# kmurf1999/RustSolver

Measured on NVIDIA B200. Metric: cfr_iterations_per_sec, higher is better.
Workload: dtype f32

## Files before the change

rustsolver_b200/csrc/kernels.cu:

```cuda
#include "kernels.cuh"

#ifndef RS_MIN_BLOCKS_288
#define RS_MIN_BLOCKS_288 3
#endif
#ifndef RS_MIN_BLOCKS_352
#define RS_MIN_BLOCKS_352 2
#endif

#ifndef RS_POLL_SLEEP_NS
#define RS_POLL_SLEEP_NS 64
#endif

namespace rs {

namespace {

__device__ __forceinline__ uint32_t ld_acquire_u32(const uint32_t* p) {
    uint32_t v;
    asm volatile("ld.acquire.gpu.global.u32 %0, [%1];" : "=r"(v) : "l"(p) : "memory");
    return v;
}
__device__ __forceinline__ uint32_t ld_acquire_sys_u32(const uint32_t* p) {
    uint32_t v;
    asm volatile("ld.acquire.sys.global.u32 %0, [%1];" : "=r"(v) : "l"(p) : "memory");
// ... 42 lines not shown
        : "=r"(ok)
        : "r"(uint32_t(__cvta_generic_to_shared(bar))), "r"(parity)
        : "memory");
    return ok != 0;
}

__device__ __forceinline__ bool wait_gives_up(const TaskArgs& A, unsigned long long t_start, uint32_t& spins) {
    if ((++spins & 255u) != 0) return false;
    if (*reinterpret_cast<const volatile unsigned int*>(&A.ctl->abort)) return true;
    bool trip = false;
    if ((spins & 4095u) == 0 && A.host_abort && *A.host_abort) trip = true;
    if (A.wait_timeout_ns) {
        unsigned long long now;
        asm volatile("mov.u64 %0, %globaltimer;" : "=l"(now));
        if (now - t_start > A.wait_timeout_ns) trip = true;
    }
    if (trip) atomicExch(&A.ctl->abort, 1u);
    return trip;
}
__device__ __forceinline__ unsigned long long global_ns() {
    unsigned long long now;
    asm volatile("mov.u64 %0, %globaltimer;" : "=l"(now));
    return now;
}

struct Ctx {
    int nc;
    int tid, lane, warp, nwarps;
    int pos4;
    int p, o, Hp, Ho, HpP, HoP, Hx;
};

constexpr int HCAP = MAX_TASK_THREADS * 4;
extern __shared__ __align__(16) float smem_raw[];
#define SM_RS (smem_raw)
#define SM_P (smem_raw + HCAP)
#define SM_GB (smem_raw + 2 * HCAP + 4)
#define SM_WSA (smem_raw + 4 * HCAP + 12)
#define SM_WSB (smem_raw + 4 * HCAP + 44)
#define SM_B (smem_raw + 4 * HCAP + 76)
#define SM_REC (reinterpret_cast<uint32_t*>(smem_raw + 4 * HCAP + 140))
#define SM_CL (reinterpret_cast<uint32_t*>(smem_raw + 8 * HCAP + 140))
#define SM_X (smem_raw + 9 * HCAP + 140)

__device__ __forceinline__ void stage_lists_raw(int tid, int HoP, const uint16_t* __restrict__ cl_pos_b) {
    if (8 * tid < 2 * HoP)
        asm volatile("cp.async.cg.shared.global [%0], [%1], 16;" ::"r"(uint32_t(__cvta_generic_to_shared(SM_CL + 4 * tid))), "l"(cl_pos_b + 8 * tid)
                     : "memory");
    asm volatile("cp.async.commit_group;" ::: "memory");
}

__device__ __forceinline__ float scan_reach(const Ctx& c, const float* r) {
    csync(c.nc);
    float4 x = f4zero();
    if (c.pos4 < c.HoP) x = *reinterpret_cast<const float4*>(r + c.pos4);
    float y[8];
    uint32_t w[4];
    {
        asm volatile("cp.async.wait_group 0;" ::: "memory");
        uint4 u = make_uint4(0x07ff07ffu, 0x07ff07ffu, 0x07ff07ffu, 0x07ff07ffu);
        if (8 * c.tid < 2 * c.HoP) u = *reinterpret_cast<const uint4*>(SM_CL + 4 * c.tid);
        w[0] = u.x;
        w[1] = u.y;
        w[2] = u.z;
        w[3] = u.w;
#pragma unroll
        for (int i = 0; i < 4; ++i) {
            const uint32_t a = w[i] & CL_POS_MASK, b = (w[i] >> 16) & CL_POS_MASK;
            y[2 * i] = a != CL_POS_NONE ? r[a] : 0.f;
            y[2 * i + 1] = b != CL_POS_NONE ? r[b] : 0.f;
        }
    }
    const float la = (x.x + x.y) + (x.z + x.w);
    float lb = 0.f;
#pragma unroll
    for (int i = 0; i < 8; ++i) lb += y[i];
    float ia = la, ib = lb;
#pragma unroll
    for (int d = 1; d < 32; d <<= 1) {
        const float ta = __shfl_up_sync(0xffffffffu, ia, d);
        const float tb = __shfl_up_sync(0xffffffffu, ib, d);
        if (c.lane >= d) {
            ia += ta;
            ib += tb;
        }
    }
    if (c.lane == 31) {
        SM_WSA[c.warp] = ia;
        SM_WSB[c.warp] = ib;
    }
    csync(c.nc);
    float wa = c.lane < c.nwarps ? SM_WSA[c.lane] : 0.f;
    float wb = c.lane < c.nwarps ? SM_WSB[c.lane] : 0.f;
#pragma unroll
    for (int d = 1; d < 16; d <<= 1) {
        const float ta = __shfl_up_sync(0xffffffffu, wa, d);
        const float tb = __shfl_up_sync(0xffffffffu, wb, d);
        if (c.lane >= d) {
            wa += ta;
            wb += tb;
        }
    }
    const float total = __shfl_sync(0xffffffffu, wa, c.nwarps - 1);
    const float total_b = __shfl_sync(0xffffffffu, wb, c.nwarps - 1);
    const float base_a = c.warp > 0 ? __shfl_sync(0xffffffffu, wa, c.warp - 1) : 0.f;
    const float base_b = c.warp > 0 ? __shfl_sync(0xffffffffu, wb, c.warp - 1) : 0.f;
    float ea = base_a + ia - la, eb = base_b + ib - lb;
    if (c.pos4 < c.HoP) {
        float4 o;
        o.x = ea;
        o.y = ea + x.x;
        o.z = o.y + x.y;
        o.w = o.z + x.z;
        *reinterpret_cast<float4*>(SM_P + c.pos4) = o;
    }
    if (8 * c.tid < 2 * c.HoP) {
        float4 o0, o1;
        o0.x = eb;
        o0.y = o0.x + y[0];
        o0.z = o0.y + y[1];
        o0.w = o0.z + y[2];
        o1.x = o0.w + y[3];
        o1.y = o1.x + y[4];
        o1.z = o1.y + y[5];
        o1.w = o1.z + y[6];
        *reinterpret_cast<float4*>(SM_GB + 8 * c.tid) = o0;
        *reinterpret_cast<float4*>(SM_GB + 8 * c.tid + 4) = o1;
        const uint32_t ord0 = ((w[0] >> 11) & 7u) | (((w[0] >> 27) & 7u) << 3);
        float* bp = SM_B + (c.tid == 0 ? 0u : ord0);
        const float ex[8] = {o0.x, o0.y, o0.z, o0.w, o1.x, o1.y, o1.z, o1.w};
#pragma unroll
        for (int i = 0; i < 8; ++i) {
            const bool first = ((w[i >> 1] >> ((i & 1) * 16)) & CL_FIRST) != 0;
            if (first) *bp++ = ex[i];
        }
        if (c.tid == 0) SM_B[ord0] = total_b;
    }
    if (c.tid == 0) {
        SM_P[c.HoP] = total;
        SM_GB[2 * c.HoP] = total_b;
    }
    csync(c.nc);
    return total;
}

__device__ __forceinline__ void load_recs4(const uint32_t* __restrict__ planes, int HpP, int pos4, uint4 (&rec)[4]) {
    const uint4 w0 = __ldg(reinterpret_cast<const uint4*>(planes + pos4));
    const uint4 w1 = __ldg(reinterpret_cast<const uint4*>(planes + HpP + pos4));
    const uint4 w2 = __ldg(reinterpret_cast<const uint4*>(planes + 2 * HpP + pos4));
    const uint4 w3 = __ldg(reinterpret_cast<const uint4*>(planes + 3 * HpP + pos4));
    rec[0] = make_uint4(w0.x, w1.x, w2.x, w3.x);
    rec[1] = make_uint4(w0.y, w1.y, w2.y, w3.y);
    rec[2] = make_uint4(w0.z, w1.z, w2.z, w3.z);
    rec[3] = make_uint4(w0.w, w1.w, w2.w, w3.w);
}

__device__ __forceinline__ void stage_recs(const Ctx& c, const uint32_t* __restrict__ planes) {
    if (c.pos4 < c.HpP) {
#pragma unroll
        for (int w = 0; w < 4; ++w)
            asm volatile("cp.async.cg.shared.global [%0], [%1], 16;" ::"r"(uint32_t(__cvta_generic_to_shared(SM_REC + w * HCAP + c.pos4))),
                         "l"(planes + size_t(w) * c.HpP + c.pos4)
                         : "memory");
    }
    asm volatile("cp.async.commit_group;" ::: "memory");
}
__device__ __forceinline__ void staged_recs_wait() { asm volatile("cp.async.wait_group 0;" ::: "memory"); }
__device__ __forceinline__ void staged_recs4(const Ctx& c, uint4 (&rec)[4]) {
    const uint4 w0 = *reinterpret_cast<const uint4*>(SM_REC + c.pos4);
    const uint4 w1 = *reinterpret_cast<const uint4*>(SM_REC + HCAP + c.pos4);
    const uint4 w2 = *reinterpret_cast<const uint4*>(SM_REC + 2 * HCAP + c.pos4);
    const uint4 w3 = *reinterpret_cast<const uint4*>(SM_REC + 3 * HCAP + c.pos4);
    rec[0] = make_uint4(w0.x, w1.x, w2.x, w3.x);
    rec[1] = make_uint4(w0.y, w1.y, w2.y, w3.y);
    rec[2] = make_uint4(w0.z, w1.z, w2.z, w3.z);
    rec[3] = make_uint4(w0.w, w1.w, w2.w, w3.w);
}

__device__ __forceinline__ float ldsb(const float* base, uint32_t byte_off) {
    return *reinterpret_cast<const float*>(reinterpret_cast<const char*>(base) + byte_off);
}
__device__ __forceinline__ void hand_terms(const Ctx& c, const float* r, float total, const uint4& rec, float& mass, float& sd) {
    const uint32_t k0 = rec.w & 0x1ffu, k1 = (rec.w >> 9) & 0x1ffu, same4 = rec.w >> 18;
    const float g0s = ldsb(SM_B, k0), g0e = ldsb(SM_B + 1, k0), g1s = ldsb(SM_B, k1), g1e = ldsb(SM_B + 1, k1);
    mass = total - (g0e - g0s) - (g1e - g1s) + (same4 != HREC_SAME_NONE ? ldsb(r, same4) : 0.f);
    sd = ldsb(SM_P, rec.x & 0xffffu) + ldsb(SM_P, rec.x >> 16) - total - ldsb(SM_GB, rec.y & 0xffffu) - ldsb(SM_GB, rec.y >> 16) + g0s + g0e -
         ldsb(SM_GB, rec.z & 0xffffu) - ldsb(SM_GB, rec.z >> 16) + g1s + g1e;
}
__device__ __forceinline__ float hand_mass(const Ctx& c, const float* r, float total, const uint4& rec) {
    const uint32_t k0 = rec.w & 0x1ffu, k1 = (rec.w >> 9) & 0x1ffu, same4 = rec.w >> 18;
    return total - (ldsb(SM_B + 1, k0) - ldsb(SM_B, k0)) - (ldsb(SM_B + 1, k1) - ldsb(SM_B, k1)) + (same4 != HREC_SAME_NONE ? ldsb(r, same4) : 0.f);
}

__device__ __forceinline__ float4 load_reach4(const TaskArgs& A, const Ctx& c, const NodeTask& nt, const RoundArgs& Rk, int k, int b) {
    float4 r = f4zero();
    if (c.pos4 >= c.HoP) return r;
    if (nt.r_in == RIN_INITIAL) {
        const uint32_t nl = Rk.rp[c.o].n_live[b];
        uint32_t s[4];
        unpack4(__ldg(reinterpret_cast<const uint2*>(Rk.rp[c.o].slot_of_pos + size_t(b) * c.HoP + c.pos4)), s);
        const float* __restrict__ w = A.root_weights[c.o];
#pragma unroll
        for (int i = 0; i < 4; ++i) f4set(r, i, uint32_t(c.pos4 + i) < nl ? __ldg(w + s[i]) : 0.f);
    } else if (nt.rin_parent_round) {
        const RoundArgs& Rp = A.rounds[k - 1];
        const float* src = Rp.rbuf + (size_t(nt.r_in) * Rp.n_boards + Rk.parent_board[b]) * c.HoP;
        uint32_t pp[4];
        unpack4(__ldg(reinterpret_cast<const uint2*>(Rk.rp[c.o].parent_pos + size_t(b) * c.HoP + c.pos4)), pp);
#pragma unroll
        for (int i = 0; i < 4; ++i) f4set(r, i, pp[i] != 0xffffu ? __ldcg(src + pp[i]) : 0.f);
    } else {
        r = ldcg4(Rk.rbuf + (size_t(nt.r_in) * Rk.n_boards + b) * c.HoP + c.pos4);
    }
    return r;
}

__device__ __forceinline__ float4 child_value4(const TaskArgs& A, const Ctx& c, const RoundArgs& Rk, const TaskChild& ch, int b) {
    float4 v = f4zero();
    if (c.pos4 >= c.HpP) return v;
    for (int s = 0; s < ch.n_src; ++s) {
        const TaskSrc sr = A.srcs[ch.src_first + s];
        const float* base = (sr.kind == SK_CBUF ? Rk.cbuf : Rk.gathered) + (size_t(sr.buf) * Rk.n_boards + b) * c.HpP;
        v = f4add(v, ldcg4(base + c.pos4));
    }
// ... 46 lines not shown
                g[4 * v + 1] = t.y;
                g[4 * v + 2] = t.z;
                g[4 * v + 3] = t.w;
            }
        } else {
#pragma unroll
            for (int e = 0; e < 4 * NA; ++e) g[e] = 0.f;
        }
    } else {
#pragma unroll
        for (int i = 0; i < 4; ++i)
#pragma unroll
            for (int a = 0; a < NA; ++a) g[i * NA + a] = rows[i] != 0xffffu ? slab[size_t(rows[i]) * NA + a] : 0.f;
    }
}

template <int NA>
__device__ __forceinline__ void xs_pick(const TaskArgs& A, float u, float (&sg)[NA]) {
    int pick = NA - 1;
    bool found = false;
    float cum = 0.f;
#pragma unroll
    for (int a = 0; a + 1 < NA; ++a) {
        cum += sg[a];
        if (!found && u < cum) {
            pick = a;
            found = true;
        }
    }
#pragma unroll
    for (int a = 0; a < NA; ++a) sg[a] = (a == pick) ? (A.xs_mode == 2 ? sg[a] : 1.0f) : 0.f;
}

template <int MODE, int NA, bool XS>
__device__ __forceinline__ void task_down(const TaskArgs& A, const Ctx& c, const NodeTask& nt, const RoundArgs& Rk, int k, int b) {
    const DevRoundPlayer& O = Rk.rp[c.o];
    const uint32_t nrp = O.n_rows_pad[b];
    const float* __restrict__ slab = (MODE == KM_CFR ? O.regrets : O.ssum) + O.board_off[b] + size_t(nrp) * nt.cum_a;
    if (nt.out >= 0) {
        stage_lists_raw(c.tid, c.HoP, O.cl_pos + size_t(b) * 2 * c.HoP);
        stage_recs(c, reinterpret_cast<const uint32_t*>(Rk.rp[c.p].hrec) + size_t(b) * 4 * c.HpP);
    }
    const float4 r4 = load_reach4(A, c, nt, Rk, k, b);
    uint32_t rows[4] = {0xffffu, 0xffffu, 0xffffu, 0xffffu};
    if (!O.identity && c.pos4 < c.HoP) unpack4(__ldg(reinterpret_cast<const uint2*>(O.row_of_pos + size_t(b) * c.HoP + c.pos4)), rows);
    float g[4 * NA];
    load_rows<NA>(slab, O.identity != 0, c.pos4, nrp, rows, g);
    float4 v[NA];
    uint32_t xs_slot[4] = {0, 0, 0, 0};
    if (XS && c.pos4 < c.HoP) unpack4(__ldg(reinterpret_cast<const uint2*>(O.slot_of_pos + size_t(b) * c.HoP + c.pos4)), xs_slot);
#pragma unroll
    for (int i = 0; i < 4; ++i) {
        float sg[NA];
        sigma_row<NA>(g, i, sg);
        if (XS) xs_pick<NA>(A, xs_uniform(A.xs_key, nt.an_index, uint32_t(Rk.board_base + b), xs_slot[i]), sg);
        const float r = f4get(r4, i);
#pragma unroll
        for (int a = 0; a < NA; ++a) f4set(v[a], i, r * sg[a]);
    }
    int slot = 0;
#pragma unroll
    for (int a = 0; a < NA; ++a) {
        const int ck = nt.child[a].kind;
        if (c.pos4 < c.HoP) {
            if (ck == CK_FOLD || ck == CK_SHOWDOWN) *reinterpret_cast<float4*>(SM_X + slot * c.Hx + c.pos4) = v[a];
            else if (nt.child[a].buf >= 0) stcg4(Rk.rbuf + (size_t(nt.child[a].buf) * Rk.n_boards + b) * c.HoP + c.pos4, v[a]);
        }
        if (ck == CK_FOLD || ck == CK_SHOWDOWN) ++slot;
    }
    if (nt.out < 0) return;
    const DevRoundPlayer& Pp = Rk.rp[c.p];
    const uint32_t nl_p = Pp.n_live[b];
    const float scale = Rk.chance_scale[b];
    float4 acc = f4zero();
    slot = 0;
    for (int a = 0; a < NA; ++a) {
        const int ck = nt.child[a].kind;
        if (ck != CK_FOLD && ck != CK_SHOWDOWN) continue;
        const float* r = SM_X + slot * c.Hx;
        ++slot;
        const float cf = nt.child[a].coef * scale;
        const float total = scan_reach(c, r);
        staged_recs_wait();
        if (c.pos4 < c.HpP) {
            uint4 rec[4];
            staged_recs4(c, rec);
#pragma unroll
            for (int i = 0; i < 4; ++i) {
                if (uint32_t(c.pos4 + i) < nl_p) {
                    float m, sd;
                    if (ck == CK_FOLD) {
                        m = hand_mass(c, r, total, rec[i]);
                        f4set(acc, i, f4get(acc, i) + cf * m);
                    } else {
                        hand_terms(c, r, total, rec[i], m, sd);
                        f4set(acc, i, f4get(acc, i) + cf * sd);
                    }
                }
            }
        }
    }
    if (c.pos4 < c.HpP) stcg4(Rk.cbuf + (size_t(nt.out) * Rk.n_boards + b) * c.HpP + c.pos4, acc);
}

template <int MODE, bool XS>
__device__ __forceinline__ void task_down_generic(const TaskArgs& A, const Ctx& c, const NodeTask& nt, const RoundArgs& Rk, int k, int b) {
    const DevRoundPlayer& O = Rk.rp[c.o];
    const uint32_t nrp = O.n_rows_pad[b];
    const float* __restrict__ slab = (MODE == KM_CFR ? O.regrets : O.ssum) + O.board_off[b] + size_t(nrp) * nt.cum_a;
    const float4 r4 = load_reach4(A, c, nt, Rk, k, b);
    const int n_act = nt.n_act;
    const uint32_t nl_o = O.n_live[b];
    uint32_t rows[4] = {0xffffu, 0xffffu, 0xffffu, 0xffffu};
    if (c.pos4 < c.HoP) unpack4(__ldg(reinterpret_cast<const uint2*>(O.row_of_pos + size_t(b) * c.HoP + c.pos4)), rows);
    if (c.pos4 < c.HoP) {
        for (int i = 0; i < 4; ++i) {
            const bool live = uint32_t(c.pos4 + i) < nl_o && rows[i] != 0xffffu;
            const float r = live ? f4get(r4, i) : 0.f;
            float norm = 0.f;
            if (live)
                for (int a = 0; a < n_act; ++a) norm += fmaxf(slab[size_t(rows[i]) * n_act + a], 0.f);
            int pick = -1;
            if (XS && live) {
                const float u = xs_uniform(A.xs_key, nt.an_index, uint32_t(Rk.board_base + b), O.slot_of_pos[size_t(b) * c.HoP + c.pos4 + i]);
                pick = n_act - 1;
                float cum = 0.f;
                for (int a = 0; a + 1 < n_act; ++a) {
                    cum += norm > 0.f ? fmaxf(slab[size_t(rows[i]) * n_act + a], 0.f) / norm : 1.0f / float(n_act);
                    if (u < cum) {
                        pick = a;
                        break;
                    }
                }
            }
            int slot = 0;
            for (int a = 0; a < n_act; ++a) {
                float v = 0.f;
                if (live) v = norm > 0.f ? r * fmaxf(slab[size_t(rows[i]) * n_act + a], 0.f) / norm : r / float(n_act);
                if (XS && live) v = (a == pick) ? (A.xs_mode == 2 ? v : r) : 0.f;
                const int ck = nt.child[a].kind;
                if (ck == CK_FOLD || ck == CK_SHOWDOWN) SM_X[(slot++) * c.Hx + c.pos4 + i] = v;
                else if (nt.child[a].buf >= 0) __stcg(Rk.rbuf + (size_t(nt.child[a].buf) * Rk.n_boards + b) * c.HoP + c.pos4 + i, v);
            }
        }
    }
    if (nt.out < 0) return;
    const DevRoundPlayer& Pp = Rk.rp[c.p];
    const uint32_t nl_p = Pp.n_live[b];
    const float scale = Rk.chance_scale[b];
    stage_lists_raw(c.tid, c.HoP, O.cl_pos + size_t(b) * 2 * c.HoP);
    float4 acc = f4zero();
    uint4 rec[4];
    if (c.pos4 < c.HpP) load_recs4(reinterpret_cast<const uint32_t*>(Pp.hrec) + size_t(b) * 4 * c.HpP, c.HpP, c.pos4, rec);
    int slot = 0;
    for (int a = 0; a < n_act; ++a) {
        const int ck = nt.child[a].kind;
        if (ck != CK_FOLD && ck != CK_SHOWDOWN) continue;
        const float* r = SM_X + slot * c.Hx;
        ++slot;
        const float cf = nt.child[a].coef * scale;
        const float total = scan_reach(c, r);
        if (c.pos4 < c.HpP) {
#pragma unroll
            for (int i = 0; i < 4; ++i) {
                if (uint32_t(c.pos4 + i) < nl_p) {
                    float m, sd;
                    hand_terms(c, r, total, rec[i], m, sd);
                    f4set(acc, i, f4get(acc, i) + cf * (ck == CK_FOLD ? m : sd));
                }
            }
        }
    }
    if (c.pos4 < c.HpP) stcg4(Rk.cbuf + (size_t(nt.out) * Rk.n_boards + b) * c.HpP + c.pos4, acc);
}

__device__ __forceinline__ void trav_terms(const TaskArgs& A, const Ctx& c, const NodeTask& nt, const RoundArgs& Rk, int k, int b,
                                           bool need_sd, float4& mass, float4& sd) {
    const DevRoundPlayer& Pp = Rk.rp[c.p];
    stage_lists_raw(c.tid, c.HoP, Rk.rp[c.o].cl_pos + size_t(b) * 2 * c.HoP);
    stage_recs(c, reinterpret_cast<const uint32_t*>(Pp.hrec) + size_t(b) * 4 * c.HpP);
    const float4 r4 = load_reach4(A, c, nt, Rk, k, b);
    if (c.pos4 < c.HoP) *reinterpret_cast<float4*>(SM_RS + c.pos4) = r4;
    const float total = scan_reach(c, SM_RS);
    mass = f4zero();
    sd = f4zero();
    const uint32_t nl_p = Pp.n_live[b];
    staged_recs_wait();
    if (c.pos4 < c.HpP) {
        uint4 rec[4];
        staged_recs4(c, rec);
#pragma unroll
        for (int i = 0; i < 4; ++i) {
            if (uint32_t(c.pos4 + i) < nl_p) {
                float m, s = 0.f;
                if (need_sd) hand_terms(c, SM_RS, total, rec[i], m, s);
                else m = hand_mass(c, SM_RS, total, rec[i]);
                f4set(mass, i, m);
                f4set(sd, i, s);
            }
        }
    }
}

__device__ __forceinline__ void trav_terms_or_load(const TaskArgs& A, const Ctx& c, const NodeTask& nt, const RoundArgs& Rk, int k, int b,
                                                   bool need_sd, float4& mass, float4& sd) {
    if (!nt.pre_terms) {
        trav_terms(A, c, nt, Rk, k, b, need_sd, mass, sd);
        return;
    }
    mass = f4zero();
    sd = f4zero();
    if (c.pos4 < c.HpP) {
        const float* m = Rk.cbuf + (size_t(nt.aux) * Rk.n_boards + b) * c.HpP + c.pos4;
        mass = ldcg4(m);
        if (need_sd) sd = ldcg4(m + size_t(Rk.n_boards) * c.HpP);
    }
}

template <int MODE, int NA>
__device__ __forceinline__ void task_trav(const TaskArgs& A, const Ctx& c, const NodeTask& nt, const RoundArgs& Rk, int k, int b) {
    const DevRoundPlayer& Pp = Rk.rp[c.p];
    const float scale = Rk.chance_scale[b];
    float4 v[NA];
    bool need_sd = false;
#pragma unroll
    for (int a = 0; a < NA; ++a) {
        v[a] = f4zero();
        need_sd |= (nt.child[a].kind == CK_SHOWDOWN);
    }
// ... 199 lines not shown
    if (kind != TK_DOWN && kind != TK_UP_TRAV) return;
    const RoundArgs& Rk = A.rounds[g->round_k];
    const int b = board_of(A, g->round_k, int(tk - g->first));
    const int q = kind == TK_DOWN ? 1 - A.trav : A.trav;
    const DevRoundPlayer& D = Rk.rp[q];
    const uint32_t nrp = D.n_rows_pad[b];
    const size_t off = D.board_off[b] + size_t(nrp) * g->cum_a;
    const uint32_t bytes = nrp * uint32_t(g->n_act) * 4u;
    if (kind == TK_DOWN) {
        prefetch_l2_bulk((MODE == KM_CFR ? D.regrets : D.ssum) + off, bytes);
    } else {
        if (MODE == KM_CFR) prefetch_l2_bulk(D.regrets + off, bytes);
        if (MODE != KM_BR) prefetch_l2_bulk(D.ssum + off, bytes);
    }
}

struct TaskSlot {
    uint32_t ticket;
    uint32_t epoch;
    uint32_t xseq;
    uint32_t pad;
    NodeTask nt;
};

template <int MODE, int MAXT, int MINB, bool XS>
__global__ void __launch_bounds__(MAXT + 32, MINB) task_kernel(const __grid_constant__ TaskArgs A) {
    __shared__ __align__(16) TaskSlot s_slot[2];

    __shared__ __align__(8) uint64_t s_done;

    const int NC = blockDim.x - 32;
    const int tid = threadIdx.x;
    if (tid == 0) mbar_init(&s_done, uint32_t(NC >> 5));
    if (tid < 2) SM_B[54 + tid] = 0.f;
    __syncthreads();

    if (tid >= NC) {
        const int lane = tid - NC;
        uint32_t epoch = 0, xseq = 0;
        if (lane == 0) {
            epoch = ld_acquire_u32(&A.ctl->epoch);
            xseq = *reinterpret_cast<const volatile unsigned int*>(&A.ctl->xch_seq);
        }
        epoch = __shfl_sync(0xffffffffu, epoch, 0);
        uint32_t prev_tk = 0xffffffffu, parity = 0;
        int buf = 0;
        uint32_t tk_next = 0;
        if (lane == 0) tk_next = A.t0 + uint32_t(atomicAdd(&A.ctl->ticket, 1ull));
        tk_next = __shfl_sync(0xffffffffu, tk_next, 0);
        for (;;) {
            bool published = (prev_tk == 0xffffffffu);
            auto try_publish = [&]() {
                if (lane == 0 && !published && mbar_test(&s_done, parity)) {
#ifndef RS_NO_PUBLISH_FENCE
                    __threadfence();
#endif
                    st_release_u32(A.flags + prev_tk, epoch);
                    published = true;
                }
            };
            uint32_t tk = tk_next;
            uint32_t sl = A.t1;
            if (tk < A.t1) {
                unsigned long long pend = 0;
                if (lane == 0) pend = atomicAdd(&A.ctl->ticket, 1ull);
                sl = A.order ? __ldg(A.order + tk) : tk;
                const uint32_t j = __ldg(A.task_of_ticket + sl);
// ... 276 lines not shown
    float4* v4 = reinterpret_cast<float4*>(data);
    const size_t stride = size_t(gridDim.x) * blockDim.x;
    for (size_t i = size_t(blockIdx.x) * blockDim.x + threadIdx.x; i < n4; i += stride) {
        float4 v = v4[i];
        v.x *= d;
        v.y *= d;
        v.z *= d;
        v.w *= d;
        v4[i] = v;
    }
    if (blockIdx.x == 0 && threadIdx.x < n - n4 * 4) data[n4 * 4 + threadIdx.x] *= d;
}

__global__ void normalize_kernel(const float* __restrict__ in, float* __restrict__ out, uint32_t n_rows, uint32_t A) {
    const uint32_t row = blockIdx.x * blockDim.x + threadIdx.x;
    if (row >= n_rows) return;
    float norm = 0.f;
    for (uint32_t a = 0; a < A; ++a) norm += fmaxf(in[size_t(row) * A + a], 0.f);
    for (uint32_t a = 0; a < A; ++a)
        out[size_t(row) * A + a] = norm > 0.f ? fmaxf(in[size_t(row) * A + a], 0.f) / norm : 1.0f / float(A);
}

__global__ void unpermute_kernel(const float* __restrict__ in, const uint16_t* __restrict__ slot_of_pos, const uint32_t* __restrict__ n_live,
                                 float* __restrict__ out, uint32_t hp, uint32_t H) {
    const uint32_t b = blockIdx.y;
    const uint32_t pos = blockIdx.x * blockDim.x + threadIdx.x;
    if (pos < n_live[b]) out[size_t(b) * H + slot_of_pos[size_t(b) * hp + pos]] = in[size_t(b) * hp + pos];
}

}

size_t task_kernel_smem_bytes(int slots, int Hp_pad, int Ho_pad) {
    const int hx = Hp_pad > Ho_pad ? Hp_pad : Ho_pad;
    size_t floats = size_t(9 * HCAP + 140) + size_t(slots) * hx;
    return floats * sizeof(float);
}

template <int MAXT, int MINB>
static cudaError_t configure_for(size_t smem, int threads, int* blocks_per_sm) {
    cudaError_t e;
    e = cudaFuncSetAttribute(task_kernel<KM_CFR, MAXT, MINB, false>, cudaFuncAttributeMaxDynamicSharedMemorySize, int(smem));
    if (e != cudaSuccess) return e;
    e = cudaFuncSetAttribute(task_kernel<KM_CFR, MAXT, MINB, true>, cudaFuncAttributeMaxDynamicSharedMemorySize, int(smem));
    if (e != cudaSuccess) return e;
    e = cudaFuncSetAttribute(task_kernel<KM_BR, MAXT, MINB, false>, cudaFuncAttributeMaxDynamicSharedMemorySize, int(smem));
    if (e != cudaSuccess) return e;
    e = cudaFuncSetAttribute(task_kernel<KM_EVAL, MAXT, MINB, false>, cudaFuncAttributeMaxDynamicSharedMemorySize, int(smem));
    if (e != cudaSuccess) return e;
    int n = 0, m = 0, x = 0;
    e = cudaOccupancyMaxActiveBlocksPerMultiprocessor(&n, task_kernel<KM_CFR, MAXT, MINB, false>, threads + 32, smem);
    if (e != cudaSuccess) return e;
    e = cudaOccupancyMaxActiveBlocksPerMultiprocessor(&m, task_kernel<KM_BR, MAXT, MINB, false>, threads + 32, smem);
    if (e != cudaSuccess) return e;
    e = cudaOccupancyMaxActiveBlocksPerMultiprocessor(&x, task_kernel<KM_CFR, MAXT, MINB, true>, threads + 32, smem);
    if (e != cudaSuccess) return e;
    n = n < x ? n : x;
    *blocks_per_sm = n < m ? n : m;
    return cudaSuccess;
}

cudaError_t configure_task_kernels(size_t smem, int threads, bool wide, int* blocks_per_sm) {
    if (threads <= 288 && !wide) return configure_for<288, RS_MIN_BLOCKS_288>(smem, threads, blocks_per_sm);
    return configure_for<352, RS_MIN_BLOCKS_352>(smem, threads, blocks_per_sm);
}

template <int MAXT, int MINB>
static void launch_for(const TaskArgs& a, int mode, int grid, int threads, size_t smem, cudaStream_t st) {
// ... 40 lines not shown
```

Measured before the change: 19.87.

## Fuse fold and showdown reach scans into one pass with paired boundary tables

When a node has exactly one fold child and one showdown child, the two prefix scans over opponent reach are done together in a single pass with four concurrent scan lanes. This saves one round of block synchronisations and one pass over the hand records. Block boundary values are now stored as duplicated pairs so each hand reads start and end with one float2 load. Scans that only feed a fold skip writing the showdown prefix arrays. In exchange, shared memory grows slightly and the scan holds more registers.

Result: no change. 19.98 (median of 6 runs) (+0.6%).

```diff
diff --git a/rustsolver_b200/csrc/kernels.cu b/rustsolver_b200/csrc/kernels.cu
--- a/rustsolver_b200/csrc/kernels.cu
+++ b/rustsolver_b200/csrc/kernels.cu
@@ -98,16 +98,21 @@
 };
 
 constexpr int HCAP = MAX_TASK_THREADS * 4;
+constexpr int B_NONE_PAIR = int(HREC_K_NONE / 4u);
 extern __shared__ __align__(16) float smem_raw[];
 #define SM_RS (smem_raw)
 #define SM_P (smem_raw + HCAP)
 #define SM_GB (smem_raw + 2 * HCAP + 4)
 #define SM_WSA (smem_raw + 4 * HCAP + 12)
 #define SM_WSB (smem_raw + 4 * HCAP + 44)
-#define SM_B (smem_raw + 4 * HCAP + 76)
-#define SM_REC (reinterpret_cast<uint32_t*>(smem_raw + 4 * HCAP + 140))
-#define SM_CL (reinterpret_cast<uint32_t*>(smem_raw + 8 * HCAP + 140))
-#define SM_X (smem_raw + 9 * HCAP + 140)
+#define SM_WSC (smem_raw + 4 * HCAP + 76)
+#define SM_WSD (smem_raw + 4 * HCAP + 108)
+#define SM_B (smem_raw + 4 * HCAP + 142)
+#define SM_BF (smem_raw + 4 * HCAP + 254)
+#define SM_REC (reinterpret_cast<uint32_t*>(smem_raw + 4 * HCAP + 364))
+#define SM_CL (reinterpret_cast<uint32_t*>(smem_raw + 8 * HCAP + 364))
+#define SM_X (smem_raw + 9 * HCAP + 364)
+constexpr int SM_FIXED_FLOATS = 9 * HCAP + 364;
 
 __device__ __forceinline__ void stage_lists_raw(int tid, int HoP, const uint16_t* __restrict__ cl_pos_b) {
     if (8 * tid < 2 * HoP)
@@ -116,10 +121,19 @@
     asm volatile("cp.async.commit_group;" ::: "memory");
 }
 
-__device__ __forceinline__ float scan_reach(const Ctx& c, const float* r) {
+__device__ __forceinline__ float list_value(const float* r, const uint32_t (&w)[4], int i) {
+    const uint32_t a = (w[i >> 1] >> ((i & 1) * 16)) & CL_POS_MASK;
+    return a != CL_POS_NONE ? r[a] : 0.f;
+}
+
+template <bool TWO>
+__device__ __forceinline__ float scan_reach_impl(const Ctx& c, const float* r, bool sd, const float* rf, float& total_f) {
     csync(c.nc);
-    float4 x = f4zero();
-    if (c.pos4 < c.HoP) x = *reinterpret_cast<const float4*>(r + c.pos4);
+    float4 x = f4zero(), xf = f4zero();
+    if (c.pos4 < c.HoP) {
+        x = *reinterpret_cast<const float4*>(r + c.pos4);
+        if (TWO) xf = *reinterpret_cast<const float4*>(rf + c.pos4);
+    }
     float y[8];
     uint32_t w[4];
     {
@@ -141,38 +155,77 @@
     float lb = 0.f;
 #pragma unroll
     for (int i = 0; i < 8; ++i) lb += y[i];
-    float ia = la, ib = lb;
+    float lc = 0.f, ld = 0.f;
+    if (TWO) {
+        lc = (xf.x + xf.y) + (xf.z + xf.w);
+#pragma unroll
+        for (int i = 0; i < 8; ++i) ld += list_value(rf, w, i);
+    }
+    float ia = la, ib = lb, ic = lc, id = ld;
 #pragma unroll
     for (int d = 1; d < 32; d <<= 1) {
         const float ta = __shfl_up_sync(0xffffffffu, ia, d);
         const float tb = __shfl_up_sync(0xffffffffu, ib, d);
+        float tc = 0.f, td = 0.f;
+        if (TWO) {
+            tc = __shfl_up_sync(0xffffffffu, ic, d);
+            td = __shfl_up_sync(0xffffffffu, id, d);
+        }
         if (c.lane >= d) {
             ia += ta;
             ib += tb;
+            if (TWO) {
+                ic += tc;
+                id += td;
+            }
         }
     }
     if (c.lane == 31) {
         SM_WSA[c.warp] = ia;
         SM_WSB[c.warp] = ib;
+        if (TWO) {
+            SM_WSC[c.warp] = ic;
+            SM_WSD[c.warp] = id;
+        }
     }
     csync(c.nc);
     float wa = c.lane < c.nwarps ? SM_WSA[c.lane] : 0.f;
     float wb = c.lane < c.nwarps ? SM_WSB[c.lane] : 0.f;
+    float wc = 0.f, wd = 0.f;
+    if (TWO) {
+        wc = c.lane < c.nwarps ? SM_WSC[c.lane] : 0.f;
+        wd = c.lane < c.nwarps ? SM_WSD[c.lane] : 0.f;
+    }
 #pragma unroll
     for (int d = 1; d < 16; d <<= 1) {
         const float ta = __shfl_up_sync(0xffffffffu, wa, d);
         const float tb = __shfl_up_sync(0xffffffffu, wb, d);
+        float tc = 0.f, td = 0.f;
+        if (TWO) {
+            tc = __shfl_up_sync(0xffffffffu, wc, d);
+            td = __shfl_up_sync(0xffffffffu, wd, d);
+        }
         if (c.lane >= d) {
             wa += ta;
             wb += tb;
+            if (TWO) {
+                wc += tc;
+                wd += td;
+            }
         }
     }
     const float total = __shfl_sync(0xffffffffu, wa, c.nwarps - 1);
     const float total_b = __shfl_sync(0xffffffffu, wb, c.nwarps - 1);
     const float base_a = c.warp > 0 ? __shfl_sync(0xffffffffu, wa, c.warp - 1) : 0.f;
     const float base_b = c.warp > 0 ? __shfl_sync(0xffffffffu, wb, c.warp - 1) : 0.f;
+    float total_d = 0.f, base_d = 0.f;
+    if (TWO) {
+        total_f = __shfl_sync(0xffffffffu, wc, c.nwarps - 1);
+        total_d = __shfl_sync(0xffffffffu, wd, c.nwarps - 1);
+        base_d = c.warp > 0 ? __shfl_sync(0xffffffffu, wd, c.warp - 1) : 0.f;
+    }
     float ea = base_a + ia - la, eb = base_b + ib - lb;
-    if (c.pos4 < c.HoP) {
+    if (sd && c.pos4 < c.HoP) {
         float4 o;
         o.x = ea;
         o.y = ea + x.x;
@@ -190,24 +243,57 @@
         o1.y = o1.x + y[4];
         o1.z = o1.y + y[5];
         o1.w = o1.z + y[6];
-        *reinterpret_cast<float4*>(SM_GB + 8 * c.tid) = o0;
-        *reinterpret_cast<float4*>(SM_GB + 8 * c.tid + 4) = o1;
+        if (sd) {
+            *reinterpret_cast<float4*>(SM_GB + 8 * c.tid) = o0;
+            *reinterpret_cast<float4*>(SM_GB + 8 * c.tid + 4) = o1;
+        }
         const uint32_t ord0 = ((w[0] >> 11) & 7u) | (((w[0] >> 27) & 7u) << 3);
-        float* bp = SM_B + (c.tid == 0 ? 0u : ord0);
-        const float ex[8] = {o0.x, o0.y, o0.z, o0.w, o1.x, o1.y, o1.z, o1.w};
-#pragma unroll
-        for (int i = 0; i < 8; ++i) {
-            const bool first = ((w[i >> 1] >> ((i & 1) * 16)) & CL_FIRST) != 0;
-            if (first) *bp++ = ex[i];
-        }
-        if (c.tid == 0) SM_B[ord0] = total_b;
-    }
-    if (c.tid == 0) {
+        const uint32_t o2 = 2u * (c.tid == 0 ? 0u : ord0);
+        {
+            float* bp = SM_B + o2;
+            const float ex[8] = {o0.x, o0.y, o0.z, o0.w, o1.x, o1.y, o1.z, o1.w};
+#pragma unroll
+            for (int i = 0; i < 8; ++i) {
+                const bool first = ((w[i >> 1] >> ((i & 1) * 16)) & CL_FIRST) != 0;
+                if (first) {
+                    bp[0] = ex[i];
+                    bp[-1] = ex[i];
+                    bp += 2;
+                }
+            }
+            if (c.tid == 0) SM_B[2 * int(ord0) - 1] = total_b;
+        }
+        if (TWO) {
+            float ex[8];
+            ex[0] = base_d + id - ld;
+#pragma unroll
+            for (int i = 1; i < 8; ++i) ex[i] = ex[i - 1] + list_value(rf, w, i - 1);
+            float* bp = SM_BF + o2;
+#pragma unroll
+            for (int i = 0; i < 8; ++i) {
+                const bool first = ((w[i >> 1] >> ((i & 1) * 16)) & CL_FIRST) != 0;
+                if (first) {
+                    bp[0] = ex[i];
+                    bp[-1] = ex[i];
+                    bp += 2;
+                }
+            }
+            if (c.tid == 0) SM_BF[2 * int(ord0) - 1] = total_d;
+        }
+    }
+    if (sd && c.tid == 0) {
         SM_P[c.HoP] = total;
         SM_GB[2 * c.HoP] = total_b;
     }
     csync(c.nc);
     return total;
+}
+__device__ __forceinline__ float scan_reach(const Ctx& c, const float* r, bool sd) {
+    float unused;
+    return scan_reach_impl<false>(c, r, sd, nullptr, unused);
+}
+__device__ __forceinline__ float scan_reach2(const Ctx& c, const float* r, const float* rf, float& total_f) {
+    return scan_reach_impl<true>(c, r, true, rf, total_f);
 }
 
 __device__ __forceinline__ void load_recs4(const uint32_t* __restrict__ planes, int HpP, int pos4, uint4 (&rec)[4]) {
@@ -246,16 +332,25 @@
 __device__ __forceinline__ float ldsb(const float* base, uint32_t byte_off) {
     return *reinterpret_cast<const float*>(reinterpret_cast<const char*>(base) + byte_off);
 }
+__device__ __forceinline__ float2 ldsb2(const float* base, uint32_t byte_off) {
+    return *reinterpret_cast<const float2*>(reinterpret_cast<const char*>(base) + byte_off);
+}
+__device__ __forceinline__ uint32_t pair_off0(const uint4& rec) { return (rec.w & 0x1ffu) << 1; }
+__device__ __forceinline__ uint32_t pair_off1(const uint4& rec) { return (rec.w >> 8) & 0x3feu; }
+__device__ __forceinline__ float mass_of(const float* r, float total, float2 g0, float2 g1, uint32_t same4) {
+    return total - (g0.y - g0.x) - (g1.y - g1.x) + (same4 != HREC_SAME_NONE ? ldsb(r, same4) : 0.f);
+}
+__device__ __forceinline__ float showdown_of(float total, const uint4& rec, float2 g0, float2 g1) {
+    return ldsb(SM_P, rec.x & 0xffffu) + ldsb(SM_P, rec.x >> 16) - total - ldsb(SM_GB, rec.y & 0xffffu) - ldsb(SM_GB, rec.y >> 16) + g0.x + g0.y -
+           ldsb(SM_GB, rec.z & 0xffffu) - ldsb(SM_GB, rec.z >> 16) + g1.x + g1.y;
+}
 __device__ __forceinline__ void hand_terms(const Ctx& c, const float* r, float total, const uint4& rec, float& mass, float& sd) {
-    const uint32_t k0 = rec.w & 0x1ffu, k1 = (rec.w >> 9) & 0x1ffu, same4 = rec.w >> 18;
-    const float g0s = ldsb(SM_B, k0), g0e = ldsb(SM_B + 1, k0), g1s = ldsb(SM_B, k1), g1e = ldsb(SM_B + 1, k1);
-    mass = total - (g0e - g0s) - (g1e - g1s) + (same4 != HREC_SAME_NONE ? ldsb(r, same4) : 0.f);
-    sd = ldsb(SM_P, rec.x & 0xffffu) + ldsb(SM_P, rec.x >> 16) - total - ldsb(SM_GB, rec.y & 0xffffu) - ldsb(SM_GB, rec.y >> 16) + g0s + g0e -
-         ldsb(SM_GB, rec.z & 0xffffu) - ldsb(SM_GB, rec.z >> 16) + g1s + g1e;
+    const float2 g0 = ldsb2(SM_B, pair_off0(rec)), g1 = ldsb2(SM_B, pair_off1(rec));
+    mass = mass_of(r, total, g0, g1, rec.w >> 18);
+    sd = showdown_of(total, rec, g0, g1);
 }
 __device__ __forceinline__ float hand_mass(const Ctx& c, const float* r, float total, const uint4& rec) {
-    const uint32_t k0 = rec.w & 0x1ffu, k1 = (rec.w >> 9) & 0x1ffu, same4 = rec.w >> 18;
-    return total - (ldsb(SM_B + 1, k0) - ldsb(SM_B, k0)) - (ldsb(SM_B + 1, k1) - ldsb(SM_B, k1)) + (same4 != HREC_SAME_NONE ? ldsb(r, same4) : 0.f);
+    return mass_of(r, total, ldsb2(SM_B, pair_off0(rec)), ldsb2(SM_B, pair_off1(rec)), rec.w >> 18);
 }
 
 __device__ __forceinline__ float4 load_reach4(const TaskArgs& A, const Ctx& c, const NodeTask& nt, const RoundArgs& Rk, int k, int b) {
@@ -409,14 +504,24 @@
     const uint32_t nl_p = Pp.n_live[b];
     const float scale = Rk.chance_scale[b];
     float4 acc = f4zero();
-    slot = 0;
+    int n_fold = 0, n_sd = 0, a_fold = 0, a_sd = 0;
+#pragma unroll
     for (int a = 0; a < NA; ++a) {
         const int ck = nt.child[a].kind;
-        if (ck != CK_FOLD && ck != CK_SHOWDOWN) continue;
-        const float* r = SM_X + slot * c.Hx;
-        ++slot;
-        const float cf = nt.child[a].coef * scale;
-        const float total = scan_reach(c, r);
+        if (ck == CK_FOLD) {
+            ++n_fold;
+            a_fold = a;
+        } else if (ck == CK_SHOWDOWN) {
+            ++n_sd;
+            a_sd = a;
+        }
+    }
+    if (n_fold == 1 && n_sd == 1) {
+        const bool fold_first = a_fold < a_sd;
+        float total_f;
+        const float total = scan_reach2(c, SM_X + (fold_first ? c.Hx : 0), SM_X + (fold_first ? 0 : c.Hx), total_f);
+        const float* rf = SM_X + (fold_first ? 0 : c.Hx);
+        const float cf_fold = nt.child[a_fold].coef * scale, cf_sd = nt.child[a_sd].coef * scale;
         staged_recs_wait();
         if (c.pos4 < c.HpP) {
             uint4 rec[4];
@@ -424,13 +529,45 @@
 #pragma unroll
             for (int i = 0; i < 4; ++i) {
                 if (uint32_t(c.pos4 + i) < nl_p) {
-                    float m, sd;
-                    if (ck == CK_FOLD) {
-                        m = hand_mass(c, r, total, rec[i]);
-                        f4set(acc, i, f4get(acc, i) + cf * m);
+                    const uint32_t k0 = pair_off0(rec[i]), k1 = pair_off1(rec[i]);
+                    const float m = mass_of(rf, total_f, ldsb2(SM_BF, k0), ldsb2(SM_BF, k1), rec[i].w >> 18);
+                    const float sd = showdown_of(total, rec[i], ldsb2(SM_B, k0), ldsb2(SM_B, k1));
+                    float t = f4get(acc, i);
+                    if (fold_first) {
+                        t = t + cf_fold * m;
+                        t = t + cf_sd * sd;
                     } else {
-                        hand_terms(c, r, total, rec[i], m, sd);
-                        f4set(acc, i, f4get(acc, i) + cf * sd);
+                        t = t + cf_sd * sd;
+                        t = t + cf_fold * m;
+                    }
+                    f4set(acc, i, t);
+                }
+            }
+        }
+    } else {
+        slot = 0;
+        for (int a = 0; a < NA; ++a) {
+            const int ck = nt.child[a].kind;
+            if (ck != CK_FOLD && ck != CK_SHOWDOWN) continue;
+            const float* r = SM_X + slot * c.Hx;
+            ++slot;
+            const float cf = nt.child[a].coef * scale;
+            const float total = scan_reach(c, r, ck == CK_SHOWDOWN);
+            staged_recs_wait();
+            if (c.pos4 < c.HpP) {
+                uint4 rec[4];
+                staged_recs4(c, rec);
+#pragma unroll
+                for (int i = 0; i < 4; ++i) {
+                    if (uint32_t(c.pos4 + i) < nl_p) {
+                        float m, sd;
+                        if (ck == CK_FOLD) {
+                            m = hand_mass(c, r, total, rec[i]);
+                            f4set(acc, i, f4get(acc, i) + cf * m);
+                        } else {
+                            hand_terms(c, r, total, rec[i], m, sd);
+                            f4set(acc, i, f4get(acc, i) + cf * sd);
+                        }
                     }
                 }
             }
@@ -495,7 +632,7 @@
         const float* r = SM_X + slot * c.Hx;
         ++slot;
         const float cf = nt.child[a].coef * scale;
-        const float total = scan_reach(c, r);
+        const float total = scan_reach(c, r, true);
         if (c.pos4 < c.HpP) {
 #pragma unroll
             for (int i = 0; i < 4; ++i) {
@@ -517,7 +654,7 @@
     stage_recs(c, reinterpret_cast<const uint32_t*>(Pp.hrec) + size_t(b) * 4 * c.HpP);
     const float4 r4 = load_reach4(A, c, nt, Rk, k, b);
     if (c.pos4 < c.HoP) *reinterpret_cast<float4*>(SM_RS + c.pos4) = r4;
-    const float total = scan_reach(c, SM_RS);
+    const float total = scan_reach(c, SM_RS, need_sd);
     mass = f4zero();
     sd = f4zero();
     const uint32_t nl_p = Pp.n_live[b];
@@ -796,7 +933,7 @@
     const int NC = blockDim.x - 32;
     const int tid = threadIdx.x;
     if (tid == 0) mbar_init(&s_done, uint32_t(NC >> 5));
-    if (tid < 2) SM_B[54 + tid] = 0.f;
+    if (tid < 4) (tid < 2 ? SM_B : SM_BF)[2 * B_NONE_PAIR + (tid & 1)] = 0.f;
     __syncthreads();
 
     if (tid >= NC) {
@@ -1139,7 +1276,7 @@
 
 size_t task_kernel_smem_bytes(int slots, int Hp_pad, int Ho_pad) {
     const int hx = Hp_pad > Ho_pad ? Hp_pad : Ho_pad;
-    size_t floats = size_t(9 * HCAP + 140) + size_t(slots) * hx;
+    size_t floats = size_t(SM_FIXED_FLOATS) + size_t(slots) * hx;
     return floats * sizeof(float);
 }
 
```

## Fuse fold and showdown reach scans into a single prefix-scan pass

Applied to the files above, without the earlier changes.

When a node has exactly one fold child and one showdown child, both reach vectors are now prefix-scanned together in one scan_reach pass, which carries the extra fold sums through the same shuffles and block syncs. The fold hand mass is then computed from separate shared buffers (SM_WSC/WSD/BF), so one full scan with its barriers is saved per such node. The terminal logic is factored into a shared down_terminals routine, and the variable-action path now stages hand records into shared memory with cp.async instead of loading them directly from global. The cost is extra registers and a slightly larger shared-memory footprint, which could affect occupancy.

After: 19.86 before, 20.60 after (median of 6 runs). 3.7% higher.

```diff
diff --git a/rustsolver_b200/csrc/kernels.cu b/rustsolver_b200/csrc/kernels.cu
--- a/rustsolver_b200/csrc/kernels.cu
+++ b/rustsolver_b200/csrc/kernels.cu
@@ -105,9 +105,12 @@
 #define SM_WSA (smem_raw + 4 * HCAP + 12)
 #define SM_WSB (smem_raw + 4 * HCAP + 44)
 #define SM_B (smem_raw + 4 * HCAP + 76)
-#define SM_REC (reinterpret_cast<uint32_t*>(smem_raw + 4 * HCAP + 140))
-#define SM_CL (reinterpret_cast<uint32_t*>(smem_raw + 8 * HCAP + 140))
-#define SM_X (smem_raw + 9 * HCAP + 140)
+#define SM_WSC (smem_raw + 4 * HCAP + 140)
+#define SM_WSD (smem_raw + 4 * HCAP + 172)
+#define SM_BF (smem_raw + 4 * HCAP + 204)
+#define SM_REC (reinterpret_cast<uint32_t*>(smem_raw + 4 * HCAP + 268))
+#define SM_CL (reinterpret_cast<uint32_t*>(smem_raw + 8 * HCAP + 268))
+#define SM_X (smem_raw + 9 * HCAP + 268)
 
 __device__ __forceinline__ void stage_lists_raw(int tid, int HoP, const uint16_t* __restrict__ cl_pos_b) {
     if (8 * tid < 2 * HoP)
@@ -116,11 +119,19 @@
     asm volatile("cp.async.commit_group;" ::: "memory");
 }
 
-__device__ __forceinline__ float scan_reach(const Ctx& c, const float* r) {
+template <bool FOLD>
+__device__ __forceinline__ float scan_reach(const Ctx& c, const float* r, const float* rf = nullptr, float* total_f = nullptr) {
     csync(c.nc);
     float4 x = f4zero();
-    if (c.pos4 < c.HoP) x = *reinterpret_cast<const float4*>(r + c.pos4);
-    float y[8];
+    float lc = 0.f;
+    if (c.pos4 < c.HoP) {
+        x = *reinterpret_cast<const float4*>(r + c.pos4);
+        if (FOLD) {
+            const float4 xf = *reinterpret_cast<const float4*>(rf + c.pos4);
+            lc = (xf.x + xf.y) + (xf.z + xf.w);
+        }
+    }
+    float y[8], yf[8];
     uint32_t w[4];
     {
         asm volatile("cp.async.wait_group 0;" ::: "memory");
@@ -135,36 +146,70 @@
             const uint32_t a = w[i] & CL_POS_MASK, b = (w[i] >> 16) & CL_POS_MASK;
             y[2 * i] = a != CL_POS_NONE ? r[a] : 0.f;
             y[2 * i + 1] = b != CL_POS_NONE ? r[b] : 0.f;
+            if (FOLD) {
+                yf[2 * i] = a != CL_POS_NONE ? rf[a] : 0.f;
+                yf[2 * i + 1] = b != CL_POS_NONE ? rf[b] : 0.f;
+            }
         }
     }
     const float la = (x.x + x.y) + (x.z + x.w);
-    float lb = 0.f;
-#pragma unroll
-    for (int i = 0; i < 8; ++i) lb += y[i];
-    float ia = la, ib = lb;
+    float lb = 0.f, ld = 0.f;
+#pragma unroll
+    for (int i = 0; i < 8; ++i) {
+        lb += y[i];
+        if (FOLD) ld += yf[i];
+    }
+    float ia = la, ib = lb, ic = lc, id = ld;
 #pragma unroll
     for (int d = 1; d < 32; d <<= 1) {
         const float ta = __shfl_up_sync(0xffffffffu, ia, d);
         const float tb = __shfl_up_sync(0xffffffffu, ib, d);
+        float tc = 0.f, td = 0.f;
+        if (FOLD) {
+            tc = __shfl_up_sync(0xffffffffu, ic, d);
+            td = __shfl_up_sync(0xffffffffu, id, d);
+        }
         if (c.lane >= d) {
             ia += ta;
             ib += tb;
+            if (FOLD) {
+                ic += tc;
+                id += td;
+            }
         }
     }
     if (c.lane == 31) {
         SM_WSA[c.warp] = ia;
         SM_WSB[c.warp] = ib;
+        if (FOLD) {
+            SM_WSC[c.warp] = ic;
+            SM_WSD[c.warp] = id;
+        }
     }
     csync(c.nc);
     float wa = c.lane < c.nwarps ? SM_WSA[c.lane] : 0.f;
     float wb = c.lane < c.nwarps ? SM_WSB[c.lane] : 0.f;
+    float wc = 0.f, wd = 0.f;
+    if (FOLD) {
+        wc = c.lane < c.nwarps ? SM_WSC[c.lane] : 0.f;
+        wd = c.lane < c.nwarps ? SM_WSD[c.lane] : 0.f;
+    }
 #pragma unroll
     for (int d = 1; d < 16; d <<= 1) {
         const float ta = __shfl_up_sync(0xffffffffu, wa, d);
         const float tb = __shfl_up_sync(0xffffffffu, wb, d);
+        float tc = 0.f, td = 0.f;
+        if (FOLD) {
+            tc = __shfl_up_sync(0xffffffffu, wc, d);
+            td = __shfl_up_sync(0xffffffffu, wd, d);
+        }
         if (c.lane >= d) {
             wa += ta;
             wb += tb;
+            if (FOLD) {
+                wc += tc;
+                wd += td;
+            }
         }
     }
     const float total = __shfl_sync(0xffffffffu, wa, c.nwarps - 1);
@@ -172,6 +217,13 @@
     const float base_a = c.warp > 0 ? __shfl_sync(0xffffffffu, wa, c.warp - 1) : 0.f;
     const float base_b = c.warp > 0 ? __shfl_sync(0xffffffffu, wb, c.warp - 1) : 0.f;
     float ea = base_a + ia - la, eb = base_b + ib - lb;
+    float total_d = 0.f, ed = 0.f;
+    if (FOLD) {
+        *total_f = __shfl_sync(0xffffffffu, wc, c.nwarps - 1);
+        total_d = __shfl_sync(0xffffffffu, wd, c.nwarps - 1);
+        const float base_d = c.warp > 0 ? __shfl_sync(0xffffffffu, wd, c.warp - 1) : 0.f;
+        ed = base_d + id - ld;
+    }
     if (c.pos4 < c.HoP) {
         float4 o;
         o.x = ea;
@@ -193,7 +245,8 @@
         *reinterpret_cast<float4*>(SM_GB + 8 * c.tid) = o0;
         *reinterpret_cast<float4*>(SM_GB + 8 * c.tid + 4) = o1;
         const uint32_t ord0 = ((w[0] >> 11) & 7u) | (((w[0] >> 27) & 7u) << 3);
-        float* bp = SM_B + (c.tid == 0 ? 0u : ord0);
+        const uint32_t b0 = c.tid == 0 ? 0u : ord0;
+        float* bp = SM_B + b0;
         const float ex[8] = {o0.x, o0.y, o0.z, o0.w, o1.x, o1.y, o1.z, o1.w};
 #pragma unroll
         for (int i = 0; i < 8; ++i) {
@@ -201,6 +254,17 @@
             if (first) *bp++ = ex[i];
         }
         if (c.tid == 0) SM_B[ord0] = total_b;
+        if (FOLD) {
+            float* bf = SM_BF + b0;
+            float e = ed;
+#pragma unroll
+            for (int i = 0; i < 8; ++i) {
+                const bool first = ((w[i >> 1] >> ((i & 1) * 16)) & CL_FIRST) != 0;
+                if (first) *bf++ = e;
+                e += yf[i];
+            }
+            if (c.tid == 0) SM_BF[ord0] = total_d;
+        }
     }
     if (c.tid == 0) {
         SM_P[c.HoP] = total;
@@ -208,17 +272,6 @@
     }
     csync(c.nc);
     return total;
-}
-
-__device__ __forceinline__ void load_recs4(const uint32_t* __restrict__ planes, int HpP, int pos4, uint4 (&rec)[4]) {
-    const uint4 w0 = __ldg(reinterpret_cast<const uint4*>(planes + pos4));
-    const uint4 w1 = __ldg(reinterpret_cast<const uint4*>(planes + HpP + pos4));
-    const uint4 w2 = __ldg(reinterpret_cast<const uint4*>(planes + 2 * HpP + pos4));
-    const uint4 w3 = __ldg(reinterpret_cast<const uint4*>(planes + 3 * HpP + pos4));
-    rec[0] = make_uint4(w0.x, w1.x, w2.x, w3.x);
-    rec[1] = make_uint4(w0.y, w1.y, w2.y, w3.y);
-    rec[2] = make_uint4(w0.z, w1.z, w2.z, w3.z);
-    rec[3] = make_uint4(w0.w, w1.w, w2.w, w3.w);
 }
 
 __device__ __forceinline__ void stage_recs(const Ctx& c, const uint32_t* __restrict__ planes) {
@@ -253,9 +306,9 @@
     sd = ldsb(SM_P, rec.x & 0xffffu) + ldsb(SM_P, rec.x >> 16) - total - ldsb(SM_GB, rec.y & 0xffffu) - ldsb(SM_GB, rec.y >> 16) + g0s + g0e -
          ldsb(SM_GB, rec.z & 0xffffu) - ldsb(SM_GB, rec.z >> 16) + g1s + g1e;
 }
-__device__ __forceinline__ float hand_mass(const Ctx& c, const float* r, float total, const uint4& rec) {
+__device__ __forceinline__ float hand_mass(const float* B, const float* r, float total, const uint4& rec) {
     const uint32_t k0 = rec.w & 0x1ffu, k1 = (rec.w >> 9) & 0x1ffu, same4 = rec.w >> 18;
-    return total - (ldsb(SM_B + 1, k0) - ldsb(SM_B, k0)) - (ldsb(SM_B + 1, k1) - ldsb(SM_B, k1)) + (same4 != HREC_SAME_NONE ? ldsb(r, same4) : 0.f);
+    return total - (ldsb(B + 1, k0) - ldsb(B, k0)) - (ldsb(B + 1, k1) - ldsb(B, k1)) + (same4 != HREC_SAME_NONE ? ldsb(r, same4) : 0.f);
 }
 
 __device__ __forceinline__ float4 load_reach4(const TaskArgs& A, const Ctx& c, const NodeTask& nt, const RoundArgs& Rk, int k, int b) {
@@ -368,6 +421,77 @@
     for (int a = 0; a < NA; ++a) sg[a] = (a == pick) ? (A.xs_mode == 2 ? sg[a] : 1.0f) : 0.f;
 }
 
+__device__ __forceinline__ void down_terminals(const Ctx& c, const NodeTask& nt, const RoundArgs& Rk, int b, int n_act) {
+    const uint32_t nl_p = Rk.rp[c.p].n_live[b];
+    const float scale = Rk.chance_scale[b];
+    int n_fold = 0, n_sd = 0, a_fold = 0, a_sd = 0;
+    for (int a = 0; a < n_act; ++a) {
+        const int ck = nt.child[a].kind;
+        if (ck == CK_FOLD) {
+            ++n_fold;
+            a_fold = a;
+        } else if (ck == CK_SHOWDOWN) {
+            ++n_sd;
+            a_sd = a;
+        }
+    }
+    float4 acc = f4zero();
+    if (n_fold == 1 && n_sd == 1) {
+        const bool fold_first = a_fold < a_sd;
+        const float* rf = SM_X + (fold_first ? 0 : c.Hx);
+        const float* rs = SM_X + (fold_first ? c.Hx : 0);
+        float total_f;
+        const float total = scan_reach<true>(c, rs, rf, &total_f);
+        const float cf = nt.child[a_fold].coef * scale, cs = nt.child[a_sd].coef * scale;
+        const float c0 = fold_first ? cf : cs, c1 = fold_first ? cs : cf;
+        staged_recs_wait();
+        if (c.pos4 < c.HpP) {
+            uint4 rec[4];
+            staged_recs4(c, rec);
+#pragma unroll
+            for (int i = 0; i < 4; ++i) {
+                if (uint32_t(c.pos4 + i) < nl_p) {
+                    float m_sd, sd;
+                    hand_terms(c, rs, total, rec[i], m_sd, sd);
+                    const float m = hand_mass(SM_BF, rf, total_f, rec[i]);
+                    const float t0 = fold_first ? m : sd, t1 = fold_first ? sd : m;
+                    f4set(acc, i, f4get(acc, i) + c0 * t0);
+                    f4set(acc, i, f4get(acc, i) + c1 * t1);
+                }
+            }
+        }
+    } else {
+        int slot = 0;
+        for (int a = 0; a < n_act; ++a) {
+            const int ck = nt.child[a].kind;
+            if (ck != CK_FOLD && ck != CK_SHOWDOWN) continue;
+            const float* r = SM_X + slot * c.Hx;
+            ++slot;
+            const float cf = nt.child[a].coef * scale;
+            const float total = scan_reach<false>(c, r);
+            staged_recs_wait();
+            if (c.pos4 < c.HpP) {
+                uint4 rec[4];
+                staged_recs4(c, rec);
+#pragma unroll
+                for (int i = 0; i < 4; ++i) {
+                    if (uint32_t(c.pos4 + i) < nl_p) {
+                        float m, sd;
+                        if (ck == CK_FOLD) {
+                            m = hand_mass(SM_B, r, total, rec[i]);
+                            f4set(acc, i, f4get(acc, i) + cf * m);
+                        } else {
+                            hand_terms(c, r, total, rec[i], m, sd);
+                            f4set(acc, i, f4get(acc, i) + cf * sd);
+                        }
+                    }
+                }
+            }
+        }
+    }
+    if (c.pos4 < c.HpP) stcg4(Rk.cbuf + (size_t(nt.out) * Rk.n_boards + b) * c.HpP + c.pos4, acc);
+}
+
 template <int MODE, int NA, bool XS>
 __device__ __forceinline__ void task_down(const TaskArgs& A, const Ctx& c, const NodeTask& nt, const RoundArgs& Rk, int k, int b) {
     const DevRoundPlayer& O = Rk.rp[c.o];
@@ -405,38 +529,7 @@
         if (ck == CK_FOLD || ck == CK_SHOWDOWN) ++slot;
     }
     if (nt.out < 0) return;
-    const DevRoundPlayer& Pp = Rk.rp[c.p];
-    const uint32_t nl_p = Pp.n_live[b];
-    const float scale = Rk.chance_scale[b];
-    float4 acc = f4zero();
-    slot = 0;
-    for (int a = 0; a < NA; ++a) {
-        const int ck = nt.child[a].kind;
-        if (ck != CK_FOLD && ck != CK_SHOWDOWN) continue;
-        const float* r = SM_X + slot * c.Hx;
-        ++slot;
-        const float cf = nt.child[a].coef * scale;
-        const float total = scan_reach(c, r);
-        staged_recs_wait();
-        if (c.pos4 < c.HpP) {
-            uint4 rec[4];
-            staged_recs4(c, rec);
-#pragma unroll
-            for (int i = 0; i < 4; ++i) {
-                if (uint32_t(c.pos4 + i) < nl_p) {
-                    float m, sd;
-                    if (ck == CK_FOLD) {
-                        m = hand_mass(c, r, total, rec[i]);
-                        f4set(acc, i, f4get(acc, i) + cf * m);
-                    } else {
-                        hand_terms(c, r, total, rec[i], m, sd);
-                        f4set(acc, i, f4get(acc, i) + cf * sd);
-                    }
-                }
-            }
-        }
-    }
-    if (c.pos4 < c.HpP) stcg4(Rk.cbuf + (size_t(nt.out) * Rk.n_boards + b) * c.HpP + c.pos4, acc);
+    down_terminals(c, nt, Rk, b, NA);
 }
 
 template <int MODE, bool XS>
@@ -481,33 +574,9 @@
         }
     }
     if (nt.out < 0) return;
-    const DevRoundPlayer& Pp = Rk.rp[c.p];
-    const uint32_t nl_p = Pp.n_live[b];
-    const float scale = Rk.chance_scale[b];
     stage_lists_raw(c.tid, c.HoP, O.cl_pos + size_t(b) * 2 * c.HoP);
-    float4 acc = f4zero();
-    uint4 rec[4];
-    if (c.pos4 < c.HpP) load_recs4(reinterpret_cast<const uint32_t*>(Pp.hrec) + size_t(b) * 4 * c.HpP, c.HpP, c.pos4, rec);
-    int slot = 0;
-    for (int a = 0; a < n_act; ++a) {
-        const int ck = nt.child[a].kind;
-        if (ck != CK_FOLD && ck != CK_SHOWDOWN) continue;
-        const float* r = SM_X + slot * c.Hx;
-        ++slot;
-        const float cf = nt.child[a].coef * scale;
-        const float total = scan_reach(c, r);
-        if (c.pos4 < c.HpP) {
-#pragma unroll
-            for (int i = 0; i < 4; ++i) {
-                if (uint32_t(c.pos4 + i) < nl_p) {
-                    float m, sd;
-                    hand_terms(c, r, total, rec[i], m, sd);
-                    f4set(acc, i, f4get(acc, i) + cf * (ck == CK_FOLD ? m : sd));
-                }
-            }
-        }
-    }
-    if (c.pos4 < c.HpP) stcg4(Rk.cbuf + (size_t(nt.out) * Rk.n_boards + b) * c.HpP + c.pos4, acc);
+    stage_recs(c, reinterpret_cast<const uint32_t*>(Rk.rp[c.p].hrec) + size_t(b) * 4 * c.HpP);
+    down_terminals(c, nt, Rk, b, n_act);
 }
 
 __device__ __forceinline__ void trav_terms(const TaskArgs& A, const Ctx& c, const NodeTask& nt, const RoundArgs& Rk, int k, int b,
@@ -517,7 +586,7 @@
     stage_recs(c, reinterpret_cast<const uint32_t*>(Pp.hrec) + size_t(b) * 4 * c.HpP);
     const float4 r4 = load_reach4(A, c, nt, Rk, k, b);
     if (c.pos4 < c.HoP) *reinterpret_cast<float4*>(SM_RS + c.pos4) = r4;
-    const float total = scan_reach(c, SM_RS);
+    const float total = scan_reach<false>(c, SM_RS);
     mass = f4zero();
     sd = f4zero();
     const uint32_t nl_p = Pp.n_live[b];
@@ -530,7 +599,7 @@
             if (uint32_t(c.pos4 + i) < nl_p) {
                 float m, s = 0.f;
                 if (need_sd) hand_terms(c, SM_RS, total, rec[i], m, s);
-                else m = hand_mass(c, SM_RS, total, rec[i]);
+                else m = hand_mass(SM_B, SM_RS, total, rec[i]);
                 f4set(mass, i, m);
                 f4set(sd, i, s);
             }
@@ -796,7 +865,7 @@
     const int NC = blockDim.x - 32;
     const int tid = threadIdx.x;
     if (tid == 0) mbar_init(&s_done, uint32_t(NC >> 5));
-    if (tid < 2) SM_B[54 + tid] = 0.f;
+    if (tid < 2) SM_B[54 + tid] = SM_BF[54 + tid] = 0.f;
     __syncthreads();
 
     if (tid >= NC) {
@@ -1139,7 +1208,7 @@
 
 size_t task_kernel_smem_bytes(int slots, int Hp_pad, int Ho_pad) {
     const int hx = Hp_pad > Ho_pad ? Hp_pad : Ho_pad;
-    size_t floats = size_t(9 * HCAP + 140) + size_t(slots) * hx;
+    size_t floats = size_t(9 * HCAP + 268) + size_t(slots) * hx;
     return floats * sizeof(float);
 }
 
```
